# zhiyongggggg/dct-cryptonets

Measured on AMD Instinct MI355X. Metric: encrypted images/sec, ResNet-20 DCT-24x16^2 CIFAR-10, higher is better.
Workload: dtype u64 torus + f64 FFT (one-level tiers keep 32-bit accumulators)

## Files before the change

dct-cryptonets_amd/csrc/fft_core.h:

```cpp
#pragma once
#include <stdint.h>
#include <type_traits>

#if defined(__HIPCC__)
#define HD __host__ __device__ __forceinline__
#else
#define HD inline __attribute__((always_inline))
#endif

namespace dctfhe {

struct cplx { double re, im; };

struct no_tick { template <int K> HD void at() {} };
#if defined(__HIP_DEVICE_COMPILE__) && defined(DCTFHE_PHASE_TIMERS)
struct phase_clock {
  unsigned long long last, acc[12];
  __device__ __forceinline__ void start() { for (int k = 0; k < 12; k++) acc[k] = 0; last = __builtin_amdgcn_s_memtime(); }
  template <int K> __device__ __forceinline__ void at() { const unsigned long long now = __builtin_amdgcn_s_memtime(); acc[K] += now - last; last = now; }
};
#endif

HD cplx cmk(double re, double im) { cplx c; c.re = re; c.im = im; return c; }
HD cplx cadd(cplx a, cplx b) { return cmk(a.re + b.re, a.im + b.im); }
HD cplx csub(cplx a, cplx b) { return cmk(a.re - b.re, a.im - b.im); }
HD cplx cmul(cplx a, cplx b) {
  return cmk(__builtin_fma(a.re, b.re, -(a.im * b.im)), __builtin_fma(a.re, b.im, a.im * b.re));
}
HD cplx cmulc(cplx a, cplx b) {
  return cmk(__builtin_fma(a.re, b.re, a.im * b.im), __builtin_fma(a.im, b.re, -(a.re * b.im)));
}
HD cplx csqr(cplx a) { return cmk(__builtin_fma(a.re, a.re, -(a.im * a.im)), 2.0 * a.re * a.im); }
HD cplx cfma(cplx a, cplx b, cplx acc) {
  cplx r;
  r.re = __builtin_fma(a.re, b.re, acc.re); r.re = __builtin_fma(-a.im, b.im, r.re);
  r.im = __builtin_fma(a.re, b.im, acc.im); r.im = __builtin_fma(a.im, b.re, r.im);
  return r;
}

template <int I, int E, class F>
HD void static_for(F&& f) {
  if constexpr (I < E) { f(std::integral_constant<int, I>{}); static_for<I + 1, E>(static_cast<F&&>(f)); }
}

HD double q64cos(int k) {
  constexpr double t[17] = {1.0, 0.99518472667219688624, 0.98078528040323044913, 0.95694033573220886494,
                            0.92387953251128675613, 0.88192126434835502971, 0.83146961230254523708,
                            0.77301045336273696081, 0.70710678118654752440, 0.63439328416364549822,
                            0.55557023301960222474, 0.47139673682599764856, 0.38268343236508977173,
                            0.29028467725446236764, 0.19509032201612826785, 0.09801714032956060199, 0.0};
  return t[k];
}
HD cplx root64(int k) {
  k &= 63;
  const int q = k >> 4, r = k & 15;
  const double c = q64cos(r), s = q64cos(16 - r);
  switch (q) {
    case 0: return cmk(c, s);
    case 1: return cmk(-s, c);
    case 2: return cmk(-c, -s);
    default: return cmk(s, -c);
  }
}

template <int K, int SIGN>
HD cplx mul_root64(cplx a) {
  constexpr int k = ((SIGN > 0 ? K : -K) % 64 + 64) % 64;
  if constexpr (k == 0) return a;
  else if constexpr (k == 16) return cmk(-a.im, a.re);
  else if constexpr (k == 32) return cmk(-a.re, -a.im);
  else if constexpr (k == 48) return cmk(a.im, -a.re);
  else if constexpr (k % 16 == 8) {
    constexpr double h = 0.70710678118654752440;
    if constexpr (k == 8) return cmk(h * (a.re - a.im), h * (a.re + a.im));
    else if constexpr (k == 24) return cmk(-h * (a.re + a.im), h * (a.re - a.im));
    else if constexpr (k == 40) return cmk(-h * (a.re - a.im), -h * (a.re + a.im));
    else return cmk(h * (a.re + a.im), -h * (a.re - a.im));
  } else {
    const cplx w = root64(k);
    return cmul(a, w);
  }
}

template <int R, int S, int SIGN>
struct small_dft {
  static HD void run(const cplx* x, cplx* y) {
    if constexpr (R == 1) {
      y[0] = x[0];
    } else if constexpr (R == 2) {
      const cplx a = x[0], b = x[S];
      y[0] = cadd(a, b); y[1] = csub(a, b);
    } else {
      cplx e[R / 2], o[R / 2];
      small_dft<R / 2, 2 * S, SIGN>::run(x, e);
      small_dft<R / 2, 2 * S, SIGN>::run(x + S, o);
      static_for<0, R / 2>([&](auto K) {
        constexpr int k = decltype(K)::value;
        const cplx t = mul_root64<k*(64 / R), SIGN>(o[k]);
        y[k] = cadd(e[k], t); y[k + R / 2] = csub(e[k], t);
      });
    }
  }
};

HD void fused_bf(const cplx a, const cplx b, const double tr, const double ti, cplx& p, cplx& m) {
  p.re = __builtin_fma(tr, b.re, __builtin_fma(-ti, b.im, a.re));
  p.im = __builtin_fma(tr, b.im, __builtin_fma(ti, b.re, a.im));
  m.re = __builtin_fma(2.0, a.re, -p.re);
  m.im = __builtin_fma(2.0, a.im, -p.im);
}
template <int R, int S, int LV>
struct fused_idft {
  static HD void run(const cplx* x, cplx* y, const cplx* pw, const cplx cw8) {
    static_assert(R == 2 || R == 4 || R == 8, "radix 8 passes");
    if constexpr (R == 2) {
      fused_bf(x[0], x[S], pw[LV].re, pw[LV].im, y[0], y[1]);
    } else {
      cplx e[R / 2], o[R / 2];
      fused_idft<R / 2, 2 * S, LV + 1>::run(x, e, pw, cw8);
      fused_idft<R / 2, 2 * S, LV + 1>::run(x + S, o, pw, cw8);
      const cplx c = pw[LV];
      fused_bf(e[0], o[0], c.re, c.im, y[0], y[R / 2]);
      if constexpr (R == 4) {
        fused_bf(e[1], o[1], -c.im, c.re, y[1], y[1 + R / 2]);
      } else {
        fused_bf(e[1], o[1], cw8.re, cw8.im, y[1], y[1 + R / 2]);
        fused_bf(e[2], o[2], -c.im, c.re, y[2], y[2 + R / 2]);
        fused_bf(e[3], o[3], -cw8.im, cw8.re, y[3], y[3 + R / 2]);
      }
    }
  }
};
HD void fused_idft_factors(const cplx b, cplx* pw, cplx& cw8) {
  constexpr double h = 0.70710678118654752440;
  pw[0] = cmk(b.re, -b.im);
  pw[1] = csqr(pw[0]);
  pw[2] = csqr(pw[1]);
  cw8 = cmk(h * (pw[0].re - pw[0].im), h * (pw[0].re + pw[0].im));
}

constexpr int geom_logp(int P) { return P == 16 ? 4 : P == 8 ? 3 : P == 4 ? 2 : -1; }
constexpr int geom_passes(int LOGM, int P) { return LOGM / geom_logp(P) + ((LOGM % geom_logp(P)) ? 1 : 0); }
constexpr int geom_radix(int LOGM, int P, int i) {
  return (i == geom_passes(LOGM, P) - 1 && (LOGM % geom_logp(P))) ? (1 << (LOGM % geom_logp(P))) : P;
}
constexpr int geom_weight(int LOGM, int P, int i) {
  int w = 1;
  for (int j = geom_passes(LOGM, P) - 1; j > i; j--) w *= geom_radix(LOGM, P, j);
  return w;
}
constexpr int geom_tw_offset(int LOGM, int P, int i) {
  int o = 0;
  for (int j = 0; j < i; j++) o += geom_weight(LOGM, P, j);
  return o;
}

template <int LOGM, int P>
struct fft_geom {
  static constexpr int M = 1 << LOGM;
  static_assert(geom_logp(P) > 0, "P must be 4, 8 or 16");
  static constexpr int T = M / P;
  static constexpr int S = geom_passes(LOGM, P);
  static_assert(S >= 2, "need at least two passes");
  static constexpr int radix(int i) { return geom_radix(LOGM, P, i); }
  static constexpr int weight(int i) { return geom_weight(LOGM, P, i); }
  static constexpr int tw_offset(int i) { return geom_tw_offset(LOGM, P, i); }
  static constexpr int TW_TOTAL = geom_tw_offset(LOGM, P, S - 1);
  static constexpr int TW_ELEMS = TW_TOTAL + T;
  static HD int skew(int idx) { return idx + (idx >> geom_logp(P)); }
  static HD int swz(int idx) { return (idx >> 9) * 576 + ((idx & 511) ^ ((idx >> 3) & 7)); }
  static constexpr bool swz_reader(int i) { return P == 8 && LOGM >= 10 && geom_radix(LOGM, P, i) == P && geom_weight(LOGM, P, i) >= 16; }
  template <int IR> static HD int ex(int idx) { if constexpr (swz_reader(IR)) return swz(idx); else return skew(idx); }
  static constexpr int EXCH_ELEMS = M + (M >> geom_logp(P));
};

HD int pass_base(int W, int R, int t) { return (t / W) * (W * R) + (t % W); }

template <int LOGM, int P, int I>
HD int pass_addr(int t, int j) {
  using G = fft_geom<LOGM, P>;
  constexpr int R = G::radix(I), W = G::weight(I);
  if constexpr (R == P) return pass_base(W, R, t) + j * W;
  else return P * t + j;
}

struct no_hook { HD void operator()() const {} };

template <int LOGM, int P, class Sync, class WSync, class Hook = no_hook>
HD void fft_forward(cplx* v, int t, const cplx* tw, const cplx twist, cplx* exch, Sync&& sync, WSync&& wsync, Hook&& before_last = Hook{}) {
  using G = fft_geom<LOGM, P>;
  constexpr int S = G::S;
  static_for<0, P>([&](auto J) { constexpr int j = decltype(J)::value; v[j] = mul_root64<j*(64 / (4 * P)), +1>(v[j]); });
  static_for<0, S>([&](auto I) {
    constexpr int i = decltype(I)::value;
    constexpr int R = G::radix(i);
    constexpr int W = G::weight(i);
    if constexpr (i == S - 1) before_last();
    cplx y[P];
    if constexpr (R == P) {
      small_dft<P, 1, -1>::run(v, y);
    } else {
      static_for<0, P / R>([&](auto Gp) { constexpr int g = decltype(Gp)::value; small_dft<R, 1, -1>::run(v + g * R, y + g * R); });
    }
    if constexpr (i < S - 1) {
      const cplx b = tw[G::tw_offset(i) + (t % W)];
      {
        cplx run = (i == 0) ? twist : cmk(1.0, 0.0);
        if constexpr (i == 0) y[0] = cmul(y[0], run);
        static_for<1, R>([&](auto K) { constexpr int k = decltype(K)::value; run = cmul(run, b); y[k] = cmul(y[k], run); });
      }
      if constexpr (W <= 64) wsync(); else sync();
      static_for<0, P>([&](auto J) { constexpr int j = decltype(J)::value; exch[G::template ex<i + 1>(pass_addr<LOGM, P, i>(t, j))] = y[j]; });
      if constexpr (W <= 64) wsync(); else sync();
      static_for<0, P>([&](auto J) { constexpr int j = decltype(J)::value; v[j] = exch[G::template ex<i + 1>(pass_addr<LOGM, P, i + 1>(t, j))]; });
    } else {
      static_for<0, P>([&](auto J) { constexpr int j = decltype(J)::value; v[j] = y[j]; });
    }
  });
}

template <int LOGM, int P, class Sync, class WSync>
HD void fft_inverse(cplx* v, int t, const cplx* tw, const cplx twist, cplx* exch, Sync&& sync, WSync&& wsync) {
  using G = fft_geom<LOGM, P>;
  constexpr int S = G::S;
  static_for<0, S>([&](auto Irev) {
    constexpr int i = S - 1 - decltype(Irev)::value;
    constexpr int R = G::radix(i);
    constexpr int W = G::weight(i);
    constexpr bool FUSED = i > 0 && i < S - 1 && R == P && P == 8;
    if constexpr (i < S - 1 && !FUSED) {
      const cplx b = tw[G::tw_offset(i) + (t % W)];
      {
        cplx run = (i == 0) ? twist : cmk(1.0, 0.0);
        if constexpr (i == 0) v[0] = cmulc(v[0], run);
        static_for<1, R>([&](auto K) { constexpr int k = decltype(K)::value; run = cmul(run, b); v[k] = cmulc(v[k], run); });
      }
    }
    cplx y[P];
    if constexpr (FUSED) {
      cplx pw[3], cw8;
      fused_idft_factors(tw[G::tw_offset(i) + (t % W)], pw, cw8);
      fused_idft<P, 1, 0>::run(v, y, pw, cw8);
    } else if constexpr (R == P) {
      small_dft<P, 1, +1>::run(v, y);
    } else {
      static_for<0, P / R>([&](auto Gp) { constexpr int g = decltype(Gp)::value; small_dft<R, 1, +1>::run(v + g * R, y + g * R); });
    }
    if constexpr (i > 0) {
      constexpr int Wp = G::weight(i - 1);
      static_for<0, P>([&](auto J) { constexpr int j = decltype(J)::value; exch[G::template ex<i - 1>(pass_addr<LOGM, P, i>(t, j))] = y[j]; });
      if constexpr (Wp <= 64) wsync(); else sync();
      static_for<0, P>([&](auto J) { constexpr int j = decltype(J)::value; v[j] = exch[G::template ex<i - 1>(pass_addr<LOGM, P, i - 1>(t, j))]; });
      if constexpr (Wp <= 64) wsync(); else sync();
    } else {
      static_for<0, P>([&](auto J) { constexpr int j = decltype(J)::value; v[j] = mul_root64<j*(64 / (4 * P)), -1>(y[j]); });
    }
  });
}

template <int LOGM, int P, int NP, class Sync, class WSync, class Tick = no_tick>
HD void fft_forward_n(cplx (&v)[NP][P], int t, const cplx* tw, const cplx twist, cplx* exch, Sync&& sync, WSync&& wsync, Tick&& tick = Tick{}) {
  using G = fft_geom<LOGM, P>;
  constexpr int S = G::S;
  static_for<0, NP>([&](auto U) {
    constexpr int u = decltype(U)::value;
    static_for<0, P>([&](auto J) { constexpr int j = decltype(J)::value; v[u][j] = mul_root64<j*(64 / (4 * P)), +1>(v[u][j]); });
  });
  static_for<0, S>([&](auto I) {
    constexpr int i = decltype(I)::value;
    constexpr int R = G::radix(i);
    constexpr int W = G::weight(i);
    if constexpr (i < S - 1) {
      const cplx b = tw[G::tw_offset(i) + (t % W)];
      const cplx run0 = (i == 0) ? twist : cmk(1.0, 0.0);
      if constexpr (W > 64) tick.template at<0>();
      if constexpr (W <= 64) wsync(); else sync();
      if constexpr (W > 64) tick.template at<1>();
      cplx y[NP][P];
      static_for<0, NP>([&](auto U) { constexpr int u = decltype(U)::value; small_dft<P, 1, -1>::run(v[u], y[u]); });
      {
        cplx run = run0;
        if constexpr (i == 0) static_for<0, NP>([&](auto U) { constexpr int u = decltype(U)::value; y[u][0] = cmul(y[u][0], run); });
        static_for<1, R>([&](auto K) {
          constexpr int k = decltype(K)::value;
          run = cmul(run, b);
          static_for<0, NP>([&](auto U) { constexpr int u = decltype(U)::value; y[u][k] = cmul(y[u][k], run); });
        });
      }
      static_for<0, NP>([&](auto U) {
        constexpr int u = decltype(U)::value;
        cplx* ex = exch + u * G::EXCH_ELEMS;
        static_for<0, P>([&](auto J) { constexpr int j = decltype(J)::value; ex[G::template ex<i + 1>(pass_addr<LOGM, P, i>(t, j))] = y[u][j]; });
      });
      if constexpr (W > 64) tick.template at<2>();
      if constexpr (W <= 64) wsync(); else sync();
      if constexpr (W > 64) tick.template at<3>();
      static_for<0, NP>([&](auto U) {
        constexpr int u = decltype(U)::value;
        const cplx* ex = exch + u * G::EXCH_ELEMS;
        static_for<0, P>([&](auto J) { constexpr int j = decltype(J)::value; v[u][j] = ex[G::template ex<i + 1>(pass_addr<LOGM, P, i + 1>(t, j))]; });
      });
    } else {
      static_for<0, NP>([&](auto U) {
        constexpr int u = decltype(U)::value;
        cplx y[P];
        if constexpr (R == P) {
          small_dft<P, 1, -1>::run(v[u], y);
        } else {
          static_for<0, P / R>([&](auto Gp) { constexpr int g = decltype(Gp)::value; small_dft<R, 1, -1>::run(v[u] + g * R, y + g * R); });
        }
        static_for<0, P>([&](auto J) { constexpr int j = decltype(J)::value; v[u][j] = y[j]; });
      });
    }
  });
  tick.template at<4>();
}

template <int LOGM, int P, int NP, class Sync, class WSync, class Tick = no_tick>
HD void fft_inverse_n(cplx (&v)[NP][P], int t, const cplx* tw, const cplx twist, cplx* exch, Sync&& sync, WSync&& wsync, Tick&& tick = Tick{}) {
  using G = fft_geom<LOGM, P>;
  constexpr int S = G::S;
  static_for<0, S>([&](auto Irev) {
    constexpr int i = S - 1 - decltype(Irev)::value;
    constexpr int R = G::radix(i);
    constexpr int W = G::weight(i);
    if constexpr (i > 0 && G::weight(i > 0 ? i - 1 : 0) > 64) tick.template at<6>();
    cplx b = cmk(1.0, 0.0), run0 = cmk(1.0, 0.0);
    if constexpr (i < S - 1) {
      b = tw[G::tw_offset(i) + (t % W)];
      if constexpr (i == 0) run0 = twist;
    }
    constexpr bool FUSED = i > 0 && i < S - 1 && R == P && P == 8;
    [[maybe_unused]] cplx pw[3], cw8;
    if constexpr (FUSED) fused_idft_factors(b, pw, cw8);
    if constexpr (i < S - 1 && !FUSED) {
      cplx run = run0;
      if constexpr (i == 0) static_for<0, NP>([&](auto U) { constexpr int u = decltype(U)::value; v[u][0] = cmulc(v[u][0], run); });
      static_for<1, R>([&](auto K) {
        constexpr int k = decltype(K)::value;
        run = cmul(run, b);
        static_for<0, NP>([&](auto U) { constexpr int u = decltype(U)::value; v[u][k] = cmulc(v[u][k], run); });
      });
    }
    static_for<0, NP>([&](auto U) {
      constexpr int u = decltype(U)::value;
      cplx y[P];
      if constexpr (FUSED) {
        fused_idft<P, 1, 0>::run(v[u], y, pw, cw8);
      } else if constexpr (R == P) {
        small_dft<P, 1, +1>::run(v[u], y);
      } else {
        static_for<0, P / R>([&](auto Gp) { constexpr int g = decltype(Gp)::value; small_dft<R, 1, +1>::run(v[u] + g * R, y + g * R); });
      }
      if constexpr (i > 0) {
        cplx* ex = exch + u * G::EXCH_ELEMS;
        static_for<0, P>([&](auto J) { constexpr int j = decltype(J)::value; ex[G::template ex<i - 1>(pass_addr<LOGM, P, i>(t, j))] = y[j]; });
      } else {
        static_for<0, P>([&](auto J) { constexpr int j = decltype(J)::value; v[u][j] = mul_root64<j*(64 / (4 * P)), -1>(y[j]); });
      }
    });
    if constexpr (i > 0) {
      constexpr int Wp = G::weight(i - 1);
      if constexpr (Wp > 64) tick.template at<7>();
      if constexpr (Wp <= 64) wsync(); else sync();
      if constexpr (Wp > 64) tick.template at<8>();
      static_for<0, NP>([&](auto U) {
        constexpr int u = decltype(U)::value;
        const cplx* ex = exch + u * G::EXCH_ELEMS;
        static_for<0, P>([&](auto J) { constexpr int j = decltype(J)::value; v[u][j] = ex[G::template ex<i - 1>(pass_addr<LOGM, P, i - 1>(t, j))]; });
      });
      if constexpr (Wp > 64) tick.template at<9>();
      if constexpr (Wp <= 64) wsync(); else sync();
      if constexpr (Wp > 64) tick.template at<10>();
    }
  });
}

template <int LOGM, int P>
HD int spectrum_freq(int p) {
  int k = 0, fw = 1;
  for (int i = 0; i < geom_passes(LOGM, P); i++) {
    const int W = geom_weight(LOGM, P, i), R = geom_radix(LOGM, P, i);
    k += ((p / W) % R) * fw;
    fw *= R;
  }
  return k;
}

template <int LOGM, int P>
inline void fill_twiddles(cplx* tw) {
  using G = fft_geom<LOGM, P>;
  const long double PI = 3.141592653589793238462643383279502884L;
  for (int i = 0; i + 1 < G::S; i++) {
    const int W = geom_weight(LOGM, P, i), R = geom_radix(LOGM, P, i);
    for (int m = 0; m < W; m++) {
      const long double a = -2.0L * PI * m / ((long double)W * R);
      tw[geom_tw_offset(LOGM, P, i) + m] = cmk((double)__builtin_cosl(a), (double)__builtin_sinl(a));
    }
  }
  for (int t = 0; t < G::T; t++) {
    const long double a = PI * t / (long double)(2 * G::M);
    tw[G::TW_TOTAL + t] = cmk((double)__builtin_cosl(a), (double)__builtin_sinl(a));
  }
}

HD double fract64(double x) {
#if defined(__HIP_DEVICE_COMPILE__)
  return __builtin_amdgcn_fract(x);
#else
  const double r = x - __builtin_floor(x);
  return r < 1.0 ? r : 0x1.fffffffffffffp-1;
#endif
}
HD uint32_t f64_to_torus32(double y) {
  const double x = __builtin_fma(fract64(y), 4294967296.0, 0.5);
#if defined(__HIP_DEVICE_COMPILE__)
  return (uint32_t)x;
#else
  return x >= 4294967296.0 ? 0xFFFFFFFFu : (uint32_t)x;
#endif
}
HD uint64_t f64_to_torus(double y) {
  const double x = fract64(y) * 4294967296.0;
  const uint32_t hi = (uint32_t)x;
  const uint32_t lo = (uint32_t)(fract64(x) * 4294967296.0);
  return ((uint64_t)hi << 32) | lo;
}

}
```

dct-cryptonets_amd/csrc/pbs_core.h:

```cpp
#pragma once
#include "fft_core.h"

namespace dctfhe {

#if defined(__HIP_DEVICE_COMPILE__)
#define DCTFHE_SCHED_BARRIER() __builtin_amdgcn_sched_barrier(0)
#define DCTFHE_UNIFORM(x) ((uint32_t)__builtin_amdgcn_readfirstlane((int)(x)))
#define DCTFHE_DEVICE 1
#else
#define DCTFHE_SCHED_BARRIER() ((void)0)
#define DCTFHE_UNIFORM(x) (x)
#endif

constexpr int PBS_KEY_BATCH = 4;
constexpr int PBS_PF_DIST = 2;

template <int LOGN, int K, int L, int P, int MB = 0>
struct pbs_geom {
  static constexpr int N = 1 << LOGN;
  static constexpr int LOGM = LOGN - 1;
  static constexpr int M = N / 2;
  using F = fft_geom<LOGM, P>;
  static constexpr int T = F::T;
  static constexpr int ROWS = (K + 1) * L;
  static constexpr size_t BSK_ELEMS_PER_KEYBIT = (size_t)ROWS * (K + 1) * M;
  static constexpr bool PAIR = K == 1 && L == 1;
#if defined(__HIP_DEVICE_COMPILE__)
  static_assert(!MB || F::T >= 64, "two-bit kernels assume one ciphertext per wave");
#endif
  static constexpr int KEY_BLOCKS = MB ? 3 : 1;
  static constexpr int RL = F::radix(F::S - 1);
  static constexpr int NG = P / RL;
  static constexpr int NL = (K >= 2 && L >= 2) ? 2 : (K >= 2 || L >= 3) ? 1 : 0;
  static constexpr bool ACC32 = L == 1;
  using acc_t = std::conditional_t<ACC32, uint32_t, uint64_t>;
  static constexpr int ACC_BYTES = (int)sizeof(acc_t);
  static constexpr int STAGE_BYTES = N * ACC_BYTES;
  static constexpr int EXCH_BYTES = F::EXCH_ELEMS * 16;
  static constexpr bool ALIAS = NL > 0 || PAIR;
  static_assert(!PAIR || (NL == 0 && EXCH_BYTES >= STAGE_BYTES), "pair mode stages each polynomial in its exchange buffer");
  static constexpr int STAGE_OFFSET = ALIAS ? 0 : EXCH_BYTES;
  static constexpr int SHARED_BYTES = PAIR ? 2 * EXCH_BYTES : MB ? EXCH_BYTES  : ALIAS ? (EXCH_BYTES > STAGE_BYTES ? EXCH_BYTES : STAGE_BYTES) : EXCH_BYTES + STAGE_BYTES;
  static constexpr int ACCL_BYTES = NL * N * ACC_BYTES;
  static constexpr int GROUP_BYTES = SHARED_BYTES + ACCL_BYTES;
  static constexpr bool TWIST_LDS = !(PAIR && LOGN >= 12);
  static constexpr int TW_LDS_ELEMS = TWIST_LDS ? F::TW_ELEMS : F::TW_TOTAL;
  static constexpr int ZLO = MB ? (LOGN + 2) / 2 : 0, ZHI = MB ? LOGN + 1 - ZLO : 0;
  static constexpr int ZLUT_ELEMS = MB ? (1 << ZLO) + (1 << ZHI) : 0;
  static constexpr int TW_BYTES = (TW_LDS_ELEMS + ZLUT_ELEMS) * 16;
};

template <int L>
HD void decompose(uint64_t v, int beta, int32_t* digs) {
  if constexpr (L == 1) {
    const uint32_t hi = (uint32_t)(v >> 32) + (1u << (31 - beta));
    digs[0] = (int32_t)hi >> (32 - beta);
  } else {
    const int total = L * beta;
    const uint64_t B = 1ULL << beta, half = B >> 1, mask = B - 1;
    uint64_t offs = 0;
    static_for<0, L>([&](auto Lv) { offs |= half << (beta * decltype(Lv)::value); });
    const uint64_t x = ((v + (1ULL << (63 - total))) >> (64 - total)) + offs;
    static_for<0, L>([&](auto Lv) {
      constexpr int lev = decltype(Lv)::value;
      digs[lev] = (int32_t)((x >> (beta * (L - 1 - lev))) & mask) - (int32_t)half;
    });
  }
}

template <int L>
HD void decompose(uint32_t v, int beta, int32_t* digs) {
  static_assert(L == 1, "32-bit accumulators are for one-level tiers");
  digs[0] = (int32_t)(v + (1u << (31 - beta))) >> (32 - beta);
}

template <int L>
constexpr int packed_digit_bits() { return L <= 3 ? 16 : 32 / (L - 1); }

template <int L>
HD uint32_t pack_digits(const int32_t* dg) {
  constexpr int FB = packed_digit_bits<L>();
  static_assert((L - 1) * FB <= 32, "the deferred digits share one 32-bit word");
  uint32_t pk = 0;
  if constexpr (L <= 3) {
    if constexpr (L > 1) pk = (uint32_t)(uint16_t)(int16_t)dg[1];
    if constexpr (L > 2) pk |= (uint32_t)(uint16_t)(int16_t)dg[2] << 16;
  } else {
    static_for<1, L>([&](auto Lv) {
      constexpr int lev = decltype(Lv)::value;
      pk |= ((uint32_t)dg[lev] & ((1u << FB) - 1)) << (FB * (lev - 1));
    });
  }
  return pk;
}

template <int L, int LEV>
HD double unpack_digit(uint32_t pk) {
  constexpr int FB = packed_digit_bits<L>();
  if constexpr (L <= 3) return (double)(int16_t)(pk >> (16 * (LEV - 1)));
  else return (double)((int32_t)(pk << (32 - FB * LEV)) >> (32 - FB));
}
HD void acc_add(uint64_t& a, double d) { a += f64_to_torus(d); }
HD void acc_add(uint32_t& a, double d) { a += f64_to_torus32(d); }
HD uint64_t acc_wide(uint64_t a) { return a; }
HD uint64_t acc_wide(uint32_t a) { return (uint64_t)a << 32; }

HD uint64_t testvec_coeff(const int64_t* table, int w, int N, int j) {
  const int box = N >> w, half = box >> 1;
  const int jj = j + half;
  return (jj < N) ? (uint64_t)table[jj / box] : (uint64_t)0 - (uint64_t)table[0];
}

#if defined(__HIP_DEVICE_COMPILE__)
__device__ __constant__ const double dctfhe_cos8[8] = {1.0, 0.70710678118654752440, 0.0, -0.70710678118654752440,
                                                       -1.0, -0.70710678118654752440, 0.0, 0.70710678118654752440};
HD cplx root8(uint32_t k) { return cmk(dctfhe_cos8[k & 7], dctfhe_cos8[(k + 6) & 7]); }
#else
HD cplx root8(uint32_t k) { return root64(8 * (int)(k & 7)); }
#endif

HD const cplx* make_uniform(const cplx* p) {
#if defined(DCTFHE_DEVICE)
  const uint64_t v = (uint64_t)p;
  return reinterpret_cast<const cplx*>(((uint64_t)DCTFHE_UNIFORM((uint32_t)(v >> 32)) << 32) | DCTFHE_UNIFORM((uint32_t)v));
#else
  return p;
#endif
}
HD cplx load_uniform_base(const cplx* base, unsigned lane) {
#if defined(DCTFHE_DEVICE)
  typedef double v2d __attribute__((ext_vector_type(2)));
  const uint64_t v = (uint64_t)base;
  const uint32_t lo = DCTFHE_UNIFORM((uint32_t)v), hi = DCTFHE_UNIFORM((uint32_t)(v >> 32));
  const __attribute__((address_space(1))) v2d* g = (const __attribute__((address_space(1))) v2d*)(((uint64_t)hi << 32) | lo);
  const v2d x = g[lane];
  return cmk(x.x, x.y);
#else
  return base[lane];
#endif
}

#if defined(__HIP_DEVICE_COMPILE__) && defined(DCTFHE_PHASE_TIMERS) || defined(DCTFHE_PHASE_TIMERS) && defined(__HIPCC__)
__device__ unsigned long long dctfhe_phase_ticks[16 * 12];
#endif
struct pbs_args {
  const uint64_t* ct_small;
  int n;
  int beta;
  const cplx* bsk;
  const int64_t* table;
  int w;
  uint64_t* out;
  int D_out;
  int accumulate;
  uint64_t body_add;
  int bsk_wrap;
  const cplx* wtab;
  const cplx* zlut;
  const cplx* twist;
  int pf_rank, pf_parts;
};

template <int LOGN, int K, int L, int P, int MB = 0, class Sync, class WSync>
HD void pbs_thread(const pbs_args& A, int t, const cplx* tw, uint64_t* stage_raw, cplx* exch, uint64_t* accl_raw, uint32_t* pf_dump, Sync&& sync, WSync&& wsync) {
  using G = pbs_geom<LOGN, K, L, P, MB>;
  constexpr int N = G::N, M = G::M, T = G::T, NL = G::NL;
  using acc_t = typename G::acc_t;
  acc_t* const stage = reinterpret_cast<acc_t*>(stage_raw);
  acc_t* const accl = reinterpret_cast<acc_t*>(accl_raw);
  const int n = A.n;
  const int msh = 64 - LOGN - 2;
  const cplx twist = A.twist[t];

  constexpr int PF_LINES = (int)(G::KEY_BLOCKS * G::BSK_ELEMS_PER_KEYBIT * 16 / 128);
  constexpr int PF_ROUNDS = (PF_LINES / 8 + T - 1) / T;
  const char* pf_ptr;
  const size_t pf_step = A.bsk_wrap > 0 ? 0 : (size_t)G::KEY_BLOCKS * G::BSK_ELEMS_PER_KEYBIT * 16;
  {
    const int parts = A.pf_parts >= 8 ? A.pf_parts : PF_LINES;
    const int per = (PF_LINES + parts - 1) / parts;
    int line = A.pf_rank * per + (t < per ? t : per - 1);
    if (line > PF_LINES - 1 - (PF_ROUNDS - 1) * T) line = PF_LINES - 1 - (PF_ROUNDS - 1) * T;
    if (line < 0) line = 0;
    pf_ptr = reinterpret_cast<const char*>(A.bsk) + (size_t)PBS_PF_DIST * pf_step + (size_t)line * 128;
  }
  acc_t acc[K + 1][2 * P];
  {
    const uint32_t bt = (uint32_t)(((A.ct_small[n] >> msh) + 1) >> 1) & (2 * N - 1);
    static_for<0, K>([&](auto Pp) {
      constexpr int p = decltype(Pp)::value;
      static_for<0, 2 * P>([&](auto R) {
        constexpr int r = decltype(R)::value;
        if constexpr (p < NL) accl[p * N + t + T * r] = 0; else acc[p][r] = 0;
      });
    });
    if constexpr (NL > 0) sync();
    static_for<0, 2 * P>([&](auto R) {
      constexpr int r = decltype(R)::value;
      const uint32_t idx = ((uint32_t)(t + T * r) + bt) & (2 * N - 1);
      const uint64_t v = testvec_coeff(A.table, A.w, N, (int)(idx & (N - 1)));
      acc[K][r] = (acc_t)(((idx & N) ? (uint64_t)0 - v : v) >> (64 - 8 * G::ACC_BYTES));
    });
  }

  uint32_t ulow0 = 0;
  constexpr uint32_t USTEP = 4u * (uint32_t)(M / (P * G::RL));
  if constexpr (MB) ulow0 = (uint32_t)(1 - 4 * spectrum_freq<G::LOGM, P>(P * t)) & (2 * N - 1);

  auto zeta = [&](uint32_t m) -> cplx {
#if defined(DCTFHE_DEVICE)
    return cmul(A.zlut[(1 << G::ZLO) + (m >> G::ZLO)], A.zlut[m & ((1u << G::ZLO) - 1)]);
#else
    return A.zlut ? cmul(A.zlut[(1 << G::ZLO) + (m >> G::ZLO)], A.zlut[m & ((1u << G::ZLO) - 1)]) : A.wtab[m];
#endif
  };
#if defined(__HIP_DEVICE_COMPILE__) && defined(DCTFHE_PHASE_TIMERS)
  phase_clock tick;
  tick.start();
#else
  no_tick tick;
#endif
  for (int i = 0; i < n; i += (MB ? 2 : 1)) {
    const uint32_t a = (uint32_t)(((A.ct_small[i] >> msh) + 1) >> 1) & (2 * N - 1);
    const cplx* bsk_i = make_uniform(A.bsk + (size_t)(A.bsk_wrap > 0 ? i % A.bsk_wrap : i) * G::BSK_ELEMS_PER_KEYBIT);
    cplx out[K + 1][P];
    if constexpr (MB && !G::PAIR) {
      const uint32_t a2 = (uint32_t)(((A.ct_small[i + 1] >> msh) + 1) >> 1) & (2 * N - 1);
      const uint32_t au = DCTFHE_UNIFORM(a), a2u = DCTFHE_UNIFORM(a2);
      const uint32_t e1 = a * ulow0, e2 = a2 * ulow0;
      const cplx* key = A.bsk + (size_t)(3 * (i >> 1)) * G::BSK_ELEMS_PER_KEYBIT;
      static_for<0, K + 1>([&](auto Pp) {
        constexpr int p = decltype(Pp)::value;
        uint32_t packed[2 * P];
        double first[2 * P];
        static_for<0, 2 * P>([&](auto R) {
          constexpr int r = decltype(R)::value;
          acc_t own;
          if constexpr (p < NL) own = accl[p * N + t + T * r]; else own = acc[p][r];
          int32_t dg[L];
          decompose<L>(own, A.beta, dg);
          first[r] = (double)dg[0];
          packed[r] = pack_digits<L>(dg);
        });
        static_for<0, L>([&](auto Lv) {
          constexpr int lev = decltype(Lv)::value;
          constexpr int row = p * L + lev;
          cplx v[P];
          static_for<0, P>([&](auto J) {
            constexpr int j = decltype(J)::value;
            if constexpr (lev == 0) v[j] = cmk(first[j], first[P + j]);
            else v[j] = cmk(unpack_digit<L, lev>(packed[j]), unpack_digit<L, lev>(packed[P + j]));
          });
          fft_forward<G::LOGM, P>(v, t, tw, twist, exch, sync, wsync);
          tick.template at<4>();
          cplx zb1 = cmk(1.0, 0.0), zb2 = cmk(1.0, 0.0);
          static_for<0, P>([&](auto J) {
            constexpr int j = decltype(J)::value;
            constexpr int g = j / G::RL, jp = j % G::RL;
            if constexpr (jp == 0) {
              zb1 = zeta((e1 - au * (USTEP * (uint32_t)g)) & (2 * N - 1));
              zb2 = zeta((e2 - a2u * (USTEP * (uint32_t)g)) & (2 * N - 1));
            }
            cplx z1 = zb1, z2 = zb2;
            if constexpr (jp > 0) {
              z1 = cmul(z1, root8((0u - au * (uint32_t)jp) * (8 / G::RL)));
              z2 = cmul(z2, root8((0u - a2u * (uint32_t)jp) * (8 / G::RL)));
            }
            cplx kk[3][K + 1];
            static_for<0, 3>([&](auto Ww) {
              constexpr int w = decltype(Ww)::value;
              static_for<0, K + 1>([&](auto Q) {
                constexpr int q = decltype(Q)::value;
                kk[w][q] = load_uniform_base(key + (((size_t)w * G::ROWS * (K + 1) + (size_t)row * (K + 1) + q) * M + j * T), (unsigned)t);
              });
            });
            DCTFHE_SCHED_BARRIER();
            const cplx m1 = cmk(z1.re - 1.0, z1.im), m2 = cmk(z2.re - 1.0, z2.im);
            cplx m12 = cmul(z1, z2); m12.re -= 1.0;
            static_for<0, K + 1>([&](auto Q) {
              constexpr int q = decltype(Q)::value;
              const cplx bundle = cfma(m12, kk[2][q], cfma(m2, kk[1][q], cmul(m1, kk[0][q])));
              if constexpr (row == 0) out[q][j] = cmul(v[j], bundle); else out[q][j] = cfma(v[j], bundle, out[q][j]);
            });
            DCTFHE_SCHED_BARRIER();
          });
          tick.template at<5>();
        });
      });
    } else if constexpr (MB) {
      const uint32_t a2 = (uint32_t)(((A.ct_small[i + 1] >> msh) + 1) >> 1) & (2 * N - 1);
      const cplx* key = A.bsk + (size_t)(3 * (i >> 1)) * G::BSK_ELEMS_PER_KEYBIT;
      cplx v[2][P];
      static_for<0, 2>([&](auto Pp) {
        constexpr int p = decltype(Pp)::value;
        static_for<0, 2 * P>([&](auto R) {
          constexpr int r = decltype(R)::value;
          int32_t dg[1];
          decompose<1>(acc[p][r], A.beta, dg);
          if constexpr (r < P) v[p][r].re = (double)dg[0]; else v[p][r - P].im = (double)dg[0];
        });
      });
      fft_forward_n<G::LOGM, P, 2>(v, t, tw, twist, exch, sync, wsync, tick);
      const uint32_t au = DCTFHE_UNIFORM(a), a2u = DCTFHE_UNIFORM(a2);
      const uint32_t e1 = a * ulow0, e2 = a2 * ulow0;
      cplx zb1 = cmk(1.0, 0.0), zb2 = cmk(1.0, 0.0);
      static_for<0, P>([&](auto J) {
        constexpr int j = decltype(J)::value;
        constexpr int g = j / G::RL, jp = j % G::RL;
        if constexpr (jp == 0) {
          zb1 = zeta((e1 - au * (USTEP * (uint32_t)g)) & (2 * N - 1));
          zb2 = zeta((e2 - a2u * (USTEP * (uint32_t)g)) & (2 * N - 1));
        }
        cplx z1 = zb1, z2 = zb2;
        if constexpr (jp > 0) {
          z1 = cmul(z1, root8((0u - au * (uint32_t)jp) * (8 / G::RL)));
          z2 = cmul(z2, root8((0u - a2u * (uint32_t)jp) * (8 / G::RL)));
        }
        static_for<0, 2>([&](auto Q) {
          constexpr int q = decltype(Q)::value;
          cplx kk[3][2];
          static_for<0, 3>([&](auto Ww) {
            constexpr int w = decltype(Ww)::value;
            static_for<0, 2>([&](auto Rr) {
              constexpr int r = decltype(Rr)::value;
              kk[w][r] = load_uniform_base(key + ((size_t)((w * 2 + r) * 2 + q) * M + j * T), (unsigned)t);
            });
          });
          DCTFHE_SCHED_BARRIER();
          const cplx m1 = cmk(z1.re - 1.0, z1.im), m2 = cmk(z2.re - 1.0, z2.im);
          cplx m12 = cmul(z1, z2); m12.re -= 1.0;
          static_for<0, 2>([&](auto Rr) {
            constexpr int r = decltype(Rr)::value;
            const cplx bundle = cfma(m12, kk[2][r], cfma(m2, kk[1][r], cmul(m1, kk[0][r])));
            if constexpr (r == 0) out[q][j] = cmul(v[0][j], bundle); else out[q][j] = cfma(v[1][j], bundle, out[q][j]);
          });
        });
      });
    } else if constexpr (G::PAIR) {
      constexpr int EX = G::F::EXCH_ELEMS * (16 / G::ACC_BYTES);
      static_for<0, 2>([&](auto Pp) {
        constexpr int p = decltype(Pp)::value;
        static_for<0, 2 * P>([&](auto R) { constexpr int r = decltype(R)::value; stage[p * EX + t + T * r] = acc[p][r]; });
      });
      sync();
      cplx v[2][P];
      static_for<0, 2>([&](auto Pp) {
        constexpr int p = decltype(Pp)::value;
        static_for<0, 2 * P>([&](auto R) {
          constexpr int r = decltype(R)::value;
          const uint32_t src = ((uint32_t)(t + T * r) - a) & (2 * N - 1);
          const acc_t x = stage[p * EX + (src & (N - 1))];
          const acc_t m = (acc_t)0 - (acc_t)((src >> LOGN) & 1);
          int32_t dg[1];
          decompose<1>((acc_t)((x ^ m) - m - acc[p][r]), A.beta, dg);
          if constexpr (r < P) v[p][r].re = (double)dg[0]; else v[p][r - P].im = (double)dg[0];
        });
      });
      fft_forward_n<G::LOGM, P, 2>(v, t, tw, twist, exch, sync, wsync);
      constexpr int KB = (P > PBS_KEY_BATCH) ? PBS_KEY_BATCH : P;
      static_for<0, 2>([&](auto Q) {
        constexpr int q = decltype(Q)::value;
        static_for<0, P / KB>([&](auto Hb) {
          constexpr int j0 = decltype(Hb)::value * KB;
          cplx k0[KB], k1[KB];
          static_for<0, KB>([&](auto J) {
            constexpr int j = decltype(J)::value;
            k0[j] = load_uniform_base(bsk_i + ((size_t)(0 * 2 + q) * M + (j0 + j) * T), (unsigned)t);
            k1[j] = load_uniform_base(bsk_i + ((size_t)(1 * 2 + q) * M + (j0 + j) * T), (unsigned)t);
          });
          DCTFHE_SCHED_BARRIER();
          static_for<0, KB>([&](auto J) {
            constexpr int j = decltype(J)::value;
            out[q][j0 + j] = cfma(v[1][j0 + j], k1[j], cfma(v[0][j0 + j], k0[j], cmk(0.0, 0.0)));
          });
          DCTFHE_SCHED_BARRIER();
        });
      });
    } else {
    static_for<0, K + 1>([&](auto Q) { static_for<0, P>([&](auto J) { out[decltype(Q)::value][decltype(J)::value] = cmk(0.0, 0.0); }); });

    static_for<0, K + 1>([&](auto Pp) {
      constexpr int p = decltype(Pp)::value;
      if constexpr (p >= NL) {
        if constexpr (G::ALIAS) sync();
        static_for<0, 2 * P>([&](auto R) { constexpr int r = decltype(R)::value; stage[t + T * r] = acc[p][r]; });
        sync();
      }
      uint32_t packed[2 * P];
      double first[2 * P];
      static_for<0, 2 * P>([&](auto R) {
        constexpr int r = decltype(R)::value;
        const uint32_t src = ((uint32_t)(t + T * r) - a) & (2 * N - 1);
        acc_t x, own;
        if constexpr (p < NL) { x = accl[p * N + (src & (N - 1))]; own = accl[p * N + t + T * r]; }
        else                  { x = stage[src & (N - 1)]; own = acc[p][r]; }
        if (src & N) x = (acc_t)0 - x;
        int32_t dg[L];
        decompose<L>((acc_t)(x - own), A.beta, dg);
        first[r] = (double)dg[0];
        packed[r] = pack_digits<L>(dg);
      });
      static_for<0, L>([&](auto Lv) {
        constexpr int lev = decltype(Lv)::value;
        cplx v[P];
        static_for<0, P>([&](auto J) {
          constexpr int j = decltype(J)::value;
          if constexpr (lev == 0) v[j] = cmk(first[j], first[P + j]);
          else v[j] = cmk(unpack_digit<L, lev>(packed[j]), unpack_digit<L, lev>(packed[P + j]));
        });
        fft_forward<G::LOGM, P>(v, t, tw, twist, exch, sync, wsync);
        const cplx* row = bsk_i + (size_t)(p * L + lev) * (K + 1) * M;
        constexpr int KBW = (K >= 2 && L == 1 && G::ACC32) ? 8 : PBS_KEY_BATCH;
        constexpr int KB = (P > KBW) ? KBW : P;
        static_for<0, K + 1>([&](auto Q) {
          constexpr int q = decltype(Q)::value;
          static_for<0, P / KB>([&](auto Hb) {
            constexpr int j0 = decltype(Hb)::value * KB;
            cplx kb[KB];
            static_for<0, KB>([&](auto J) {
              constexpr int j = decltype(J)::value;
              kb[j] = load_uniform_base(row + ((size_t)q * M + (j0 + j) * T), (unsigned)t);
            });
            DCTFHE_SCHED_BARRIER();
            static_for<0, KB>([&](auto J) { constexpr int j = decltype(J)::value; out[q][j0 + j] = cfma(v[j0 + j], kb[j], out[q][j0 + j]); });
            DCTFHE_SCHED_BARRIER();
          });
        });
      });
    });
    }

    if constexpr (T > 64) {
      uint32_t acc_pf = 0;
      static_for<0, PF_ROUNDS>([&](auto Rr) { acc_pf ^= *reinterpret_cast<const uint32_t*>(pf_ptr + (size_t)decltype(Rr)::value * T * 128); });
#if defined(__HIP_DEVICE_COMPILE__)
      asm volatile("" ::"v"(acc_pf));
#else
      pf_dump[t] = acc_pf;
#endif
      pf_ptr += pf_step;
    }

    tick.template at<5>();
    if constexpr (G::PAIR) fft_inverse_n<G::LOGM, P, 2>(out, t, tw, twist, exch, sync, wsync, tick);
    static_for<0, K + 1>([&](auto Q) {
      constexpr int q = decltype(Q)::value;
      if constexpr (!G::PAIR) fft_inverse<G::LOGM, P>(out[q], t, tw, twist, exch, sync, wsync);
      static_for<0, P>([&](auto J) {
        constexpr int j = decltype(J)::value;
        if constexpr (q < NL) {
          acc_add(accl[q * N + t + T * j], out[q][j].re);
          acc_add(accl[q * N + t + T * (P + j)], out[q][j].im);
        } else {
          acc_add(acc[q][j], out[q][j].re);
          acc_add(acc[q][P + j], out[q][j].im);
        }
      });
    });
    tick.template at<11>();
  }

#if defined(__HIP_DEVICE_COMPILE__) && defined(DCTFHE_PHASE_TIMERS)
  tick.template at<0>();
  if (blockIdx.x == DCTFHE_PHASE_TIMERS && (threadIdx.x & 63) == 0)
    for (int k = 0; k < 12; k++) dctfhe_phase_ticks[(threadIdx.x >> 6) * 12 + k] = tick.acc[k];
#endif
  uint64_t* o = A.out;
  static_for<0, K>([&](auto Pp) {
    constexpr int p = decltype(Pp)::value;
    static_for<0, 2 * P>([&](auto R) {
      constexpr int r = decltype(R)::value;
      const int c = t + T * r;
      const int dst = p * N + (c == 0 ? 0 : N - c);
      uint64_t av;
      if constexpr (p < NL) av = acc_wide(accl[p * N + c]); else av = acc_wide(acc[p][r]);
      const uint64_t v = (c == 0) ? av : (uint64_t)0 - av;
      if (A.accumulate) o[dst] += v; else o[dst] = v;
    });
  });
  if (!A.accumulate)
    for (int j = K * N + t; j < A.D_out; j += T) o[j] = 0;
  if (t == 0) {
    if (A.accumulate) o[A.D_out] += acc_wide(acc[K][0]) + A.body_add; else o[A.D_out] = acc_wide(acc[K][0]) + A.body_add;
  }
}

template <int LOGN, int P, class Sync, class WSync>
HD void key_poly_to_fourier(const uint64_t* poly, cplx* dst, int t, const cplx* tw, cplx* exch, Sync&& sync, WSync&& wsync) {
  constexpr int N = 1 << LOGN, M = N / 2;
  using F = fft_geom<LOGN - 1, P>;
  constexpr int T = F::T;
  cplx v[P];
  static_for<0, P>([&](auto J) {
    constexpr int j = decltype(J)::value;
    v[j] = cmk((double)(int64_t)poly[t + T * j], (double)(int64_t)poly[t + T * j + M]);
  });
  fft_forward<LOGN - 1, P>(v, t, tw, tw[F::TW_TOTAL + t], exch, sync, wsync);
  const double inv = 0x1p-64 / (double)M;
  static_for<0, P>([&](auto J) { constexpr int j = decltype(J)::value; dst[j * T + t] = cmk(v[j].re * inv, v[j].im * inv); });
}

}
```

Measured before the change: 0.08555.

## Add fused-twiddle DIT forward FFT for radix-8 PBS tiers

Adds a decimation-in-time forward negacyclic FFT for radix 8 that folds the per-pass twiddles into fused butterflies (FMA-based, sign-parameterised fused_idft), deriving per-thread ratios from existing twiddle tables plus a small extra last-pass table. Per-parameter selection keeps the old DIF form for some tiers and uses DIT elsewhere. The aim is to cut the complex multiplies spent on the twiddle chains in the forward FFT of blind rotation. In exchange it changes the numerical path (series-based constant rotations) and adds table entries and register pressure.

```diff
diff --git a/dct-cryptonets_amd/csrc/fft_core.h b/dct-cryptonets_amd/csrc/fft_core.h
--- a/dct-cryptonets_amd/csrc/fft_core.h
+++ b/dct-cryptonets_amd/csrc/fft_core.h
@@ -109,7 +109,7 @@
   m.re = __builtin_fma(2.0, a.re, -p.re);
   m.im = __builtin_fma(2.0, a.im, -p.im);
 }
-template <int R, int S, int LV>
+template <int R, int S, int LV, int SIGN = +1>
 struct fused_idft {
   static HD void run(const cplx* x, cplx* y, const cplx* pw, const cplx cw8) {
     static_assert(R == 2 || R == 4 || R == 8, "radix 8 passes");
@@ -117,16 +117,26 @@
       fused_bf(x[0], x[S], pw[LV].re, pw[LV].im, y[0], y[1]);
     } else {
       cplx e[R / 2], o[R / 2];
-      fused_idft<R / 2, 2 * S, LV + 1>::run(x, e, pw, cw8);
-      fused_idft<R / 2, 2 * S, LV + 1>::run(x + S, o, pw, cw8);
+      fused_idft<R / 2, 2 * S, LV + 1, SIGN>::run(x, e, pw, cw8);
+      fused_idft<R / 2, 2 * S, LV + 1, SIGN>::run(x + S, o, pw, cw8);
       const cplx c = pw[LV];
       fused_bf(e[0], o[0], c.re, c.im, y[0], y[R / 2]);
-      if constexpr (R == 4) {
-        fused_bf(e[1], o[1], -c.im, c.re, y[1], y[1 + R / 2]);
+      if constexpr (SIGN > 0) {
+        if constexpr (R == 4) {
+          fused_bf(e[1], o[1], -c.im, c.re, y[1], y[1 + R / 2]);
+        } else {
+          fused_bf(e[1], o[1], cw8.re, cw8.im, y[1], y[1 + R / 2]);
+          fused_bf(e[2], o[2], -c.im, c.re, y[2], y[2 + R / 2]);
+          fused_bf(e[3], o[3], -cw8.im, cw8.re, y[3], y[3 + R / 2]);
+        }
       } else {
-        fused_bf(e[1], o[1], cw8.re, cw8.im, y[1], y[1 + R / 2]);
-        fused_bf(e[2], o[2], -c.im, c.re, y[2], y[2 + R / 2]);
-        fused_bf(e[3], o[3], -cw8.im, cw8.re, y[3], y[3 + R / 2]);
+        if constexpr (R == 4) {
+          fused_bf(e[1], o[1], c.im, -c.re, y[1], y[1 + R / 2]);
+        } else {
+          fused_bf(e[1], o[1], cw8.re, cw8.im, y[1], y[1 + R / 2]);
+          fused_bf(e[2], o[2], c.im, -c.re, y[2], y[2 + R / 2]);
+          fused_bf(e[3], o[3], cw8.im, -cw8.re, y[3], y[3 + R / 2]);
+        }
       }
     }
   }
@@ -137,6 +147,13 @@
   pw[1] = csqr(pw[0]);
   pw[2] = csqr(pw[1]);
   cw8 = cmk(h * (pw[0].re - pw[0].im), h * (pw[0].re + pw[0].im));
+}
+template <int R>
+HD void fused_fdft_factors(const cplx c, cplx* pw, cplx& cw8) {
+  constexpr double h = 0.70710678118654752440;
+  pw[0] = c;
+  if constexpr (R >= 4) pw[1] = csqr(pw[0]);
+  if constexpr (R >= 8) { pw[2] = csqr(pw[1]); cw8 = cmk(h * (c.re + c.im), h * (c.im - c.re)); }
 }
 
 constexpr int geom_logp(int P) { return P == 16 ? 4 : P == 8 ? 3 : P == 4 ? 2 : -1; }
@@ -165,7 +182,8 @@
   static constexpr int radix(int i) { return geom_radix(LOGM, P, i); }
   static constexpr int weight(int i) { return geom_weight(LOGM, P, i); }
   static constexpr int tw_offset(int i) { return geom_tw_offset(LOGM, P, i); }
-  static constexpr int TW_TOTAL = geom_tw_offset(LOGM, P, S - 1);
+  static constexpr int TW_LAST = geom_tw_offset(LOGM, P, S - 1);
+  static constexpr int TW_TOTAL = TW_LAST + (geom_radix(LOGM, P, S - 1) == 4 && P == 8 ? 4 : 0);
   static constexpr int TW_ELEMS = TW_TOTAL + T;
   static HD int skew(int idx) { return idx + (idx >> geom_logp(P)); }
   static HD int swz(int idx) { return (idx >> 9) * 576 + ((idx & 511) ^ ((idx >> 3) & 7)); }
@@ -187,7 +205,7 @@
 struct no_hook { HD void operator()() const {} };
 
 template <int LOGM, int P, class Sync, class WSync, class Hook = no_hook>
-HD void fft_forward(cplx* v, int t, const cplx* tw, const cplx twist, cplx* exch, Sync&& sync, WSync&& wsync, Hook&& before_last = Hook{}) {
+HD void fft_forward_dif(cplx* v, int t, const cplx* tw, const cplx twist, cplx* exch, Sync&& sync, WSync&& wsync, Hook&& before_last = Hook{}) {
   using G = fft_geom<LOGM, P>;
   constexpr int S = G::S;
   static_for<0, P>([&](auto J) { constexpr int j = decltype(J)::value; v[j] = mul_root64<j*(64 / (4 * P)), +1>(v[j]); });
@@ -217,6 +235,140 @@
       static_for<0, P>([&](auto J) { constexpr int j = decltype(J)::value; v[j] = y[j]; });
     }
   });
+}
+
+
+enum { FWD_DIF = 0, FWD_DIT = 1 };
+constexpr int fwd_default_form(int P) { return P == 8 ? FWD_DIT : FWD_DIF; }
+
+template <int ND>
+HD int rev_digits(int h) {
+  static_assert(ND >= 1 && ND <= 3, "up to four passes");
+  if constexpr (ND == 1) return h;
+  else if constexpr (ND == 2) return ((h & 7) << 3) | (h >> 3);
+  else return ((h & 7) << 6) | (h & 56) | (h >> 6);
+}
+constexpr int geom_fweight(int LOGM, int P, int l) {
+  int F = 1;
+  for (int j = 0; j < l; j++) F *= geom_radix(LOGM, P, j);
+  return F;
+}
+constexpr int fwd_table(int LOGM, int P, int l) {
+  int i = geom_passes(LOGM, P) - 2;
+  while (i > 0 && geom_weight(LOGM, P, i) < geom_fweight(LOGM, P, l)) i--;
+  return i;
+}
+constexpr double series_cosm1(double x) { double c = 1.0; for (int k = 9; k >= 2; k--) c = 1.0 - x * x / (double)((2 * k - 1) * (2 * k)) * c; return -0.5 * x * x * c; }
+constexpr double series_sin(double x) { double s = 1.0; for (int k = 9; k >= 1; k--) s = 1.0 - x * x / (double)((2 * k) * (2 * k + 1)) * s; return x * s; }
+template <int LOGM, int P, int L_>
+HD cplx fwd_times_const(const cplx b) {
+  constexpr double a = 3.14159265358979323846 * (double)geom_weight(LOGM, P, L_) / (double)(2 << LOGM);
+  constexpr double cm1 = series_cosm1(a), sn = series_sin(a);
+  return cmk(b.re + __builtin_fma(-b.im, sn, b.re * cm1), b.im + __builtin_fma(b.re, sn, b.im * cm1));
+}
+constexpr int fwd_table4(int LOGM, int P, int l) {
+  int i = geom_passes(LOGM, P) - 2;
+  while (i >= 0 && geom_weight(LOGM, P, i) < 4 * geom_fweight(LOGM, P, l)) i--;
+  return i;
+}
+template <int LOGM, int P, int L_>
+HD cplx fwd_ratio(int t, const cplx* tw) {
+  using G = fft_geom<LOGM, P>;
+  static_assert(G::radix(L_) == P, "full-radix pass");
+  constexpr int W = G::weight(L_), FL = geom_fweight(LOGM, P, L_), T4 = fwd_table4(LOGM, P, L_);
+  const int kap = rev_digits<L_>(t / W);
+  if constexpr (T4 >= 0) {
+    constexpr int stride = G::weight(T4) / (4 * FL);
+    cplx c = tw[G::tw_offset(T4) + (kap == 0 ? 1 : 4 * kap - 1) * stride];
+    if (kap == 0) c.im = -c.im;
+    return c;
+  } else {
+    constexpr int TI = fwd_table(LOGM, P, L_), stride = G::weight(TI) / FL;
+    static_assert(stride >= 1, "pass table TI covers e^{-2 pi i kappa/(F_l P)}, kappa < F_l");
+    return fwd_times_const<LOGM, P, L_>(tw[G::tw_offset(TI) + kap * stride]);
+  }
+}
+template <int LOGM, int P>
+HD cplx fwd_last_ratio(int t, const cplx* tw) {
+  using G = fft_geom<LOGM, P>;
+  constexpr int RL = G::radix(G::S - 1);
+  static_assert(G::S >= 3, "a smaller last radix follows at least two full passes");
+  const cplx b = tw[rev_digits<G::S - 2>(t / RL)];
+  if constexpr (RL == 2) {
+    const cplx c = fwd_times_const<LOGM, P, G::S - 1>(b);
+    return (t & 1) ? cmk(c.im, -c.re) : c;
+  } else {
+    return cmul(b, tw[G::TW_LAST + (t % RL)]);
+  }
+}
+
+template <int LOGM, int P, int L_, int NP>
+HD void fwd_dit_pass(cplx (*v)[P], cplx (*y)[P], int t, const cplx* tw) {
+  using G = fft_geom<LOGM, P>;
+#if defined(__HIP_DEVICE_COMPILE__)
+  asm volatile("" : "+v"(t));
+#endif
+  constexpr int R = G::radix(L_);
+  if constexpr (R == P) {
+    const cplx c = fwd_ratio<LOGM, P, L_>(t, tw);
+    cplx e[NP][P / 2], o[NP][P / 2];
+    {
+      cplx pw[2];
+      pw[0] = csqr(c); pw[1] = csqr(pw[0]);
+      static_for<0, NP>([&](auto U) {
+        constexpr int u = decltype(U)::value;
+        fused_idft<P / 2, 2, 0, -1>::run(v[u], e[u], pw, pw[0]);
+        fused_idft<P / 2, 2, 0, -1>::run(v[u] + 1, o[u], pw, pw[0]);
+      });
+    }
+    constexpr double h = 0.70710678118654752440;
+    const cplx cw8 = cmk(h * (c.re + c.im), h * (c.im - c.re));
+    static_for<0, NP>([&](auto U) {
+      constexpr int u = decltype(U)::value;
+      fused_bf(e[u][0], o[u][0], c.re, c.im, y[u][0], y[u][4]);
+      fused_bf(e[u][1], o[u][1], cw8.re, cw8.im, y[u][1], y[u][5]);
+      fused_bf(e[u][2], o[u][2], c.im, -c.re, y[u][2], y[u][6]);
+      fused_bf(e[u][3], o[u][3], cw8.im, -cw8.re, y[u][3], y[u][7]);
+    });
+  } else {
+    const cplx c0 = fwd_last_ratio<LOGM, P>(t, tw);
+    static_for<0, P / R>([&](auto Gp) {
+      constexpr int g = decltype(Gp)::value;
+      cplx pw[3], cw8 = cmk(0.0, 0.0);
+      fused_fdft_factors<R>(mul_root64<g*(64 / (P * R)), -1>(c0), pw, cw8);
+      static_for<0, NP>([&](auto U) { constexpr int u = decltype(U)::value; fused_idft<R, 1, 0, -1>::run(v[u] + g * R, y[u] + g * R, pw, cw8); });
+    });
+  }
+}
+
+template <int LOGM, int P, class Sync, class WSync, class Hook = no_hook>
+HD void fft_forward_dit(cplx* v, int t, const cplx* tw, cplx* exch, Sync&& sync, WSync&& wsync, Hook&& before_last = Hook{}) {
+  using G = fft_geom<LOGM, P>;
+  constexpr int S = G::S;
+  static_assert(P == 8, "fused butterflies: radix 8");
+  static_for<0, P>([&](auto J) { constexpr int j = decltype(J)::value; v[j] = mul_root64<j*(64 / (4 * P)), +1>(v[j]); });
+  static_for<0, S>([&](auto I) {
+    constexpr int i = decltype(I)::value;
+    constexpr int W = G::weight(i);
+    if constexpr (i == S - 1) before_last();
+    cplx y[1][P];
+    if constexpr (i == 0) small_dft<P, 1, -1>::run(v, y[0]);
+    else fwd_dit_pass<LOGM, P, i, 1>(reinterpret_cast<cplx (*)[P]>(v), y, t, tw);
+    if constexpr (i < S - 1) {
+      if constexpr (W <= 64) wsync(); else sync();
+      static_for<0, P>([&](auto J) { constexpr int j = decltype(J)::value; exch[G::template ex<i + 1>(pass_addr<LOGM, P, i>(t, j))] = y[0][j]; });
+      if constexpr (W <= 64) wsync(); else sync();
+      static_for<0, P>([&](auto J) { constexpr int j = decltype(J)::value; v[j] = exch[G::template ex<i + 1>(pass_addr<LOGM, P, i + 1>(t, j))]; });
+    } else {
+      static_for<0, P>([&](auto J) { constexpr int j = decltype(J)::value; v[j] = y[0][j]; });
+    }
+  });
+}
+
+template <int LOGM, int P, int FORM = fwd_default_form(P), class Sync, class WSync, class Hook = no_hook>
+HD void fft_forward(cplx* v, int t, const cplx* tw, [[maybe_unused]] const cplx twist, cplx* exch, Sync&& sync, WSync&& wsync, Hook&& before_last = Hook{}) {
+  if constexpr (FORM == FWD_DIT) fft_forward_dit<LOGM, P>(v, t, tw, exch, sync, wsync, before_last);
+  else fft_forward_dif<LOGM, P>(v, t, tw, twist, exch, sync, wsync, before_last);
 }
 
 template <int LOGM, int P, class Sync, class WSync>
@@ -259,7 +411,7 @@
 }
 
 template <int LOGM, int P, int NP, class Sync, class WSync, class Tick = no_tick>
-HD void fft_forward_n(cplx (&v)[NP][P], int t, const cplx* tw, const cplx twist, cplx* exch, Sync&& sync, WSync&& wsync, Tick&& tick = Tick{}) {
+HD void fft_forward_n_dif(cplx (&v)[NP][P], int t, const cplx* tw, const cplx twist, cplx* exch, Sync&& sync, WSync&& wsync, Tick&& tick = Tick{}) {
   using G = fft_geom<LOGM, P>;
   constexpr int S = G::S;
   static_for<0, NP>([&](auto U) {
@@ -314,6 +466,56 @@
     }
   });
   tick.template at<4>();
+}
+
+template <int LOGM, int P, int NP, class Sync, class WSync, class Tick = no_tick>
+HD void fft_forward_n_dit(cplx (&v)[NP][P], int t, const cplx* tw, cplx* exch, Sync&& sync, WSync&& wsync, Tick&& tick = Tick{}) {
+  using G = fft_geom<LOGM, P>;
+  constexpr int S = G::S;
+  static_assert(P == 8, "fused butterflies: radix 8");
+  static_for<0, NP>([&](auto U) {
+    constexpr int u = decltype(U)::value;
+    static_for<0, P>([&](auto J) { constexpr int j = decltype(J)::value; v[u][j] = mul_root64<j*(64 / (4 * P)), +1>(v[u][j]); });
+  });
+  static_for<0, S>([&](auto I) {
+    constexpr int i = decltype(I)::value;
+    constexpr int W = G::weight(i);
+    if constexpr (i < S - 1) {
+      if constexpr (W > 64) tick.template at<0>();
+      if constexpr (W <= 64) wsync(); else sync();
+      if constexpr (W > 64) tick.template at<1>();
+      cplx y[NP][P];
+      if constexpr (i == 0) static_for<0, NP>([&](auto U) { constexpr int u = decltype(U)::value; small_dft<P, 1, -1>::run(v[u], y[u]); });
+      else fwd_dit_pass<LOGM, P, i, NP>(v, y, t, tw);
+      static_for<0, NP>([&](auto U) {
+        constexpr int u = decltype(U)::value;
+        cplx* ex = exch + u * G::EXCH_ELEMS;
+        static_for<0, P>([&](auto J) { constexpr int j = decltype(J)::value; ex[G::template ex<i + 1>(pass_addr<LOGM, P, i>(t, j))] = y[u][j]; });
+      });
+      if constexpr (W > 64) tick.template at<2>();
+      if constexpr (W <= 64) wsync(); else sync();
+      if constexpr (W > 64) tick.template at<3>();
+      static_for<0, NP>([&](auto U) {
+        constexpr int u = decltype(U)::value;
+        const cplx* ex = exch + u * G::EXCH_ELEMS;
+        static_for<0, P>([&](auto J) { constexpr int j = decltype(J)::value; v[u][j] = ex[G::template ex<i + 1>(pass_addr<LOGM, P, i + 1>(t, j))]; });
+      });
+    } else {
+      cplx y[NP][P];
+      fwd_dit_pass<LOGM, P, i, NP>(v, y, t, tw);
+      static_for<0, NP>([&](auto U) {
+        constexpr int u = decltype(U)::value;
+        static_for<0, P>([&](auto J) { constexpr int j = decltype(J)::value; v[u][j] = y[u][j]; });
+      });
+    }
+  });
+  tick.template at<4>();
+}
+
+template <int LOGM, int P, int NP, int FORM = fwd_default_form(P), class Sync, class WSync, class Tick = no_tick>
+HD void fft_forward_n(cplx (&v)[NP][P], int t, const cplx* tw, [[maybe_unused]] const cplx twist, cplx* exch, Sync&& sync, WSync&& wsync, Tick&& tick = Tick{}) {
+  if constexpr (FORM == FWD_DIT) fft_forward_n_dit<LOGM, P, NP>(v, t, tw, exch, sync, wsync, tick);
+  else fft_forward_n_dif<LOGM, P, NP>(v, t, tw, twist, exch, sync, wsync, tick);
 }
 
 template <int LOGM, int P, int NP, class Sync, class WSync, class Tick = no_tick>
@@ -398,6 +600,13 @@
       tw[geom_tw_offset(LOGM, P, i) + m] = cmk((double)__builtin_cosl(a), (double)__builtin_sinl(a));
     }
   }
+  if (G::TW_TOTAL > G::TW_LAST) {
+    const int RL = geom_radix(LOGM, P, G::S - 1);
+    for (int r = 0; r < RL; r++) {
+      const long double a = PI / (long double)(2 * G::M) - 2.0L * PI * r / (long double)(RL * RL);
+      tw[G::TW_LAST + r] = cmk((double)__builtin_cosl(a), (double)__builtin_sinl(a));
+    }
+  }
   for (int t = 0; t < G::T; t++) {
     const long double a = PI * t / (long double)(2 * G::M);
     tw[G::TW_TOTAL + t] = cmk((double)__builtin_cosl(a), (double)__builtin_sinl(a));
diff --git a/dct-cryptonets_amd/csrc/pbs_core.h b/dct-cryptonets_amd/csrc/pbs_core.h
--- a/dct-cryptonets_amd/csrc/pbs_core.h
+++ b/dct-cryptonets_amd/csrc/pbs_core.h
@@ -14,6 +14,13 @@
 
 constexpr int PBS_KEY_BATCH = 4;
 constexpr int PBS_PF_DIST = 2;
+
+constexpr int pbs_forward_form(int LOGN, int K, int L, int P) {
+  if (P != 8) return FWD_DIF;
+  if (K == 2 && LOGN == 10 && L == 2) return FWD_DIF;
+  if (K == 1 && (L == 2 || L == 3) && (LOGN == 11 || LOGN == 12 || (LOGN == 13 && L == 2))) return FWD_DIF;
+  return FWD_DIT;
+}
 
 template <int LOGN, int K, int L, int P, int MB = 0>
 struct pbs_geom {
@@ -48,6 +55,11 @@
   static constexpr int ZLO = MB ? (LOGN + 2) / 2 : 0, ZHI = MB ? LOGN + 1 - ZLO : 0;
   static constexpr int ZLUT_ELEMS = MB ? (1 << ZLO) + (1 << ZHI) : 0;
   static constexpr int TW_BYTES = (TW_LDS_ELEMS + ZLUT_ELEMS) * 16;
+#if defined(DCTFHE_FWD_FORM)
+  static constexpr int FWD = (P == 8) ? DCTFHE_FWD_FORM : FWD_DIF;
+#else
+  static constexpr int FWD = pbs_forward_form(LOGN, K, L, P);
+#endif
 };
 
 template <int L>
@@ -251,7 +263,7 @@
             if constexpr (lev == 0) v[j] = cmk(first[j], first[P + j]);
             else v[j] = cmk(unpack_digit<L, lev>(packed[j]), unpack_digit<L, lev>(packed[P + j]));
           });
-          fft_forward<G::LOGM, P>(v, t, tw, twist, exch, sync, wsync);
+          fft_forward<G::LOGM, P, G::FWD>(v, t, tw, twist, exch, sync, wsync);
           tick.template at<4>();
           cplx zb1 = cmk(1.0, 0.0), zb2 = cmk(1.0, 0.0);
           static_for<0, P>([&](auto J) {
@@ -300,7 +312,7 @@
           if constexpr (r < P) v[p][r].re = (double)dg[0]; else v[p][r - P].im = (double)dg[0];
         });
       });
-      fft_forward_n<G::LOGM, P, 2>(v, t, tw, twist, exch, sync, wsync, tick);
+      fft_forward_n<G::LOGM, P, 2, G::FWD>(v, t, tw, twist, exch, sync, wsync, tick);
       const uint32_t au = DCTFHE_UNIFORM(a), a2u = DCTFHE_UNIFORM(a2);
       const uint32_t e1 = a * ulow0, e2 = a2 * ulow0;
       cplx zb1 = cmk(1.0, 0.0), zb2 = cmk(1.0, 0.0);
@@ -356,7 +368,7 @@
           if constexpr (r < P) v[p][r].re = (double)dg[0]; else v[p][r - P].im = (double)dg[0];
         });
       });
-      fft_forward_n<G::LOGM, P, 2>(v, t, tw, twist, exch, sync, wsync);
+      fft_forward_n<G::LOGM, P, 2, G::FWD>(v, t, tw, twist, exch, sync, wsync);
       constexpr int KB = (P > PBS_KEY_BATCH) ? PBS_KEY_BATCH : P;
       static_for<0, 2>([&](auto Q) {
         constexpr int q = decltype(Q)::value;
@@ -408,7 +420,7 @@
           if constexpr (lev == 0) v[j] = cmk(first[j], first[P + j]);
           else v[j] = cmk(unpack_digit<L, lev>(packed[j]), unpack_digit<L, lev>(packed[P + j]));
         });
-        fft_forward<G::LOGM, P>(v, t, tw, twist, exch, sync, wsync);
+        fft_forward<G::LOGM, P, G::FWD>(v, t, tw, twist, exch, sync, wsync);
         const cplx* row = bsk_i + (size_t)(p * L + lev) * (K + 1) * M;
         constexpr int KBW = (K >= 2 && L == 1 && G::ACC32) ? 8 : PBS_KEY_BATCH;
         constexpr int KB = (P > KBW) ? KBW : P;
```

After: 0.08550. About the same (-0.1%).
